# Dunni3/keypoint-diffusion

Measured on AMD Instinct MI355X. Metric: denoising steps/sec, higher is better.
Workload: dtype f32; 1 GPU; egnn_all_atom dynamics (6 EGNN layers, hidden 256, update_kp_feat; fixed receptor encoder), batch of 64 synthetic 300-atom pockets / 25-atom ligands per GPU, T=500, seeded random-init weights, every step taken from the t=T ligand state; batch_per_gpu=64, n_rec=300, n_lig=25, parallelism=dp1

## Files before the change

### keypoint-diffusion_amd/csrc/egnn.hip

```cpp
#include <string.h>

#include <map>
#include <set>
#include <string>
#include <vector>

#include "egnn_kernels.h"
#include "egnn_wide.h"
#include "mfma_core.h"

using namespace kpd;

namespace {

struct LayerW {
    float *wp_e[4], *wx_e[4], *b_e[4], *wr_e[4], *watt[4];
    float *wp_c[4], *wx_c[4], *b_c[4], *wr_c[4], *w3[4];
    void *wh_e[4], *wh_c[4];
    void *chh_p[2][NSLOT];
    void *wh_a[2], *wh_b[2], *wh_2[2];
    float *wp_p[2][NSLOT], *wx_p[2][NSLOT], *b_p[2][NSLOT];
    float *ch_p[2][NSLOT], *wcol_p[2][NSLOT];
    float *wp_a[2], *wx_a[2], *wp_b[2], *wx_b[2], *b0[2], *wp_2[2], *wx_2[2], *b2[2], *ln_w[2], *ln_b[2];
};

const int kSrcNt[4] = {NT_LIG, NT_KP, NT_LIG, NT_KP};
const int kDstNt[4] = {NT_LIG, NT_LIG, NT_KP, NT_KP};
const int kSrcSlot[4] = {0, 0, 6, 4};
const int kDstSlot[4] = {2, 4, 2, 6};
const char *kEtName[4] = {"ll", "kl", "lk", "kk"};
const char *kNtName[2] = {"lig", "kp"};

std::vector<std::string> split(const std::string &s, char c) {
    std::vector<std::string> out;
    size_t p = 0;
    while (true) {
        size_t q = s.find(c, p);
        out.push_back(s.substr(p, q == std::string::npos ? q : q - p));
        if (q == std::string::npos) break;
        p = q + 1;
    }
    return out;
}

int et_index(const std::string &s) {
    for (int i = 0; i < 4; ++i)
        if (s == kEtName[i]) return i;
    return -1;
}
int nt_index(const std::string &s) {
    for (int i = 0; i < 2; ++i)
        if (s == kNtName[i]) return i;
    return -1;
}

}

struct kpd_egnn {
    kpd_egnn_config cfg;
    int n_et;
    int n_upd;
    bool rec_identity;
    Arena warena, ws;
    std::vector<LayerW> L;
    float *le_W0, *le_b0, *le_W1t, *le_b1;
    float *re_W0, *re_b0, *re_W1t, *re_b1;
    float *de_W0, *de_b0, *de_W1, *de_b1;
    std::set<std::string> expected, loaded;
    bool committed = false;
    int debug_layers = -1;
    bool f16_ok = true;
    float *widen_buf = nullptr;
    int *widen_map = nullptr;
    size_t widen_floats = 0, widen_ints = 0;
    int gemm_mode = 0;
    bool f32_only = false;
    int prune_last = 1;
    bool prof_on = false;
    std::vector<hipEvent_t> prof_ev;
    size_t prof_used = 0;

    int cap_B = 0, cap_lig = 0, cap_kp = 0, cap_kk = 0, cap_ll = 0, cap_kl = 0, cap_maxlig = 0, cap_maxkp = 0;
    int tile_cap = 0, tiles_et_cap[4] = {0, 0, 0, 0};
    float *h[2], *x[2], *P[2];
    float *hn_main[4], *hn_cont[4], *xn_main[4], *xn_cont[4];
    int *bidx[2];
    float *z[2];
    int *meta, *ll_deg, *ll_off, *kl_off, *kl_pg;
    kpd_lig_graph lg;
    int kp_table = 1;
    int tab_rows = 0;
    bool last_table = false;
    int *rowmap = nullptr, *kp_ok = nullptr;
    float *tab_in = nullptr;
    int *tab_bidx = nullptr;
    float *hT = nullptr, *PT = nullptr;
    EgnnWide *wide = nullptr;
};

static kpd_status build_weight_arena(kpd_egnn *m) {
    const kpd_egnn_config &c = m->cfg;
    m->warena.poison_at = 2;
    m->L.assign(c.n_layers, LayerW());
    return carve(m->warena, ARENA_TAIL, [&](Carve &A) {
        for (int i = 0; i < c.n_layers; ++i) {
            LayerW &w = m->L[i];
            const std::string pre = "egnn.conv_layers." + std::to_string(i) + ".";
            for (int et = 0; et < m->n_et; ++et) {
                A(w.wp_e[et], WP_FLOATS); A(w.wx_e[et], HS); A(w.b_e[et], HS); A(w.wr_e[et], HS); A(w.watt[et], HS);
                A(w.wp_c[et], WP_FLOATS); A(w.wx_c[et], HS); A(w.b_c[et], HS); A(w.wr_c[et], HS); A(w.w3[et], HS);
                A.as<unsigned short>(w.wh_e[et], WH_HALVES); A.as<unsigned short>(w.wh_c[et], WH_HALVES);
                for (int var = 0; var < 2; ++var) {
                    const int ss = kSrcSlot[et] + var, ds = kDstSlot[et] + var;
                    A(w.wp_p[kSrcNt[et]][ss], WP_FLOATS); A(w.wx_p[kSrcNt[et]][ss], HS);
                    A(w.wp_p[kDstNt[et]][ds], WP_FLOATS); A(w.wx_p[kDstNt[et]][ds], HS); A(w.b_p[kDstNt[et]][ds], HS);
                    A(w.ch_p[kSrcNt[et]][ss], 16 * 4096); A(w.wcol_p[kSrcNt[et]][ss], HS);
                    A(w.ch_p[kDstNt[et]][ds], 16 * 4096); A(w.wcol_p[kDstNt[et]][ds], HS);
                    A.as<unsigned short>(w.chh_p[kSrcNt[et]][ss], CHH_HALVES);
                    A.as<unsigned short>(w.chh_p[kDstNt[et]][ds], CHH_HALVES);
                }
                const std::string e = kEtName[et];
                for (const char *blk : {"edge_mlp.", "coord_mlp."})
                    for (const char *s : {".0.weight", ".0.bias", ".2.weight", ".2.bias"}) m->expected.insert(pre + blk + e + s);
                m->expected.insert(pre + "coord_mlp." + e + ".4.weight");
                m->expected.insert(pre + "soft_attention." + e + ".0.weight");
                m->expected.insert(pre + "soft_attention." + e + ".0.bias");
            }
            for (int nt = 0; nt < m->n_upd; ++nt) {
                A(w.wp_a[nt], WP_FLOATS); A(w.wx_a[nt], HS); A(w.wp_b[nt], WP_FLOATS); A(w.wx_b[nt], HS); A(w.b0[nt], HS);
                A(w.wp_2[nt], WP_FLOATS); A(w.wx_2[nt], HS); A(w.b2[nt], HS); A(w.ln_w[nt], HS); A(w.ln_b[nt], HS);
                A.as<unsigned short>(w.wh_a[nt], WH_HALVES); A.as<unsigned short>(w.wh_b[nt], WH_HALVES);
                A.as<unsigned short>(w.wh_2[nt], WH_HALVES);
                const std::string n = kNtName[nt];
                for (const char *s : {".0.weight", ".0.bias", ".2.weight", ".2.bias"}) m->expected.insert(pre + "node_mlp." + n + s);
                if (c.norm) {
                    m->expected.insert(pre + "layer_norm." + n + ".weight");
                    m->expected.insert(pre + "layer_norm." + n + ".bias");
                }
            }
        }
        A(m->le_W0, 64 * c.atom_nf); A(m->le_b0, 64);
        A(m->le_W1t, 64 * 256); A(m->le_b1, 256);
        for (const char *s : {"lig_encoder.0.weight", "lig_encoder.0.bias", "lig_encoder.2.weight", "lig_encoder.2.bias",
                              "lig_decoder.0.weight", "lig_decoder.0.bias", "lig_decoder.2.weight", "lig_decoder.2.bias"})
            m->expected.insert(s);
        if (!m->rec_identity) {
            A(m->re_W0, 2 * c.rec_nf * c.rec_nf); A(m->re_b0, 2 * c.rec_nf);
            A(m->re_W1t, 2 * c.rec_nf * 256); A(m->re_b1, 256);
            for (const char *s : {"rec_encoder.0.weight", "rec_encoder.0.bias", "rec_encoder.2.weight", "rec_encoder.2.bias"})
                m->expected.insert(s);
        } else {
            m->re_W0 = m->re_b0 = m->re_W1t = m->re_b1 = nullptr;
        }
        A(m->de_W0, 2 * c.atom_nf * 256); A(m->de_b0, 2 * c.atom_nf);
        A(m->de_W1, 2 * c.atom_nf * c.atom_nf); A(m->de_b1, c.atom_nf);
    });
}

extern "C" kpd_status kpd_egnn_create(const kpd_egnn_config *cfg, kpd_egnn **out) {
    KPD_REQUIRE(cfg && out, KPD_ERR_INVALID, "null argument");
    KPD_REQUIRE(cfg->hidden_nf >= 1 && cfg->hidden_nf <= WIDE_MAX_HID, KPD_ERR_INVALID, "hidden_nf=%d: the HIP path covers 1 .. %d",
                cfg->hidden_nf, WIDE_MAX_HID);
    KPD_REQUIRE(cfg->ll_k >= 0 && cfg->ll_k <= KL_KMAX, KPD_ERR_INVALID, "ll_k=%d outside 0..%d (0 = radius graph)", cfg->ll_k, KL_KMAX);
    KPD_REQUIRE(cfg->kl_k >= 0 && cfg->kl_k <= KL_KMAX, KPD_ERR_INVALID, "kl_k=%d outside 0..%d (0 = radius graph)", cfg->kl_k, KL_KMAX);
    KPD_REQUIRE(cfg->kl_k > 0 || cfg->kl_cutoff > 0.0f, KPD_ERR_INVALID, "kl_k = 0 needs graph_cutoffs['kl'] > 0");
    KPD_REQUIRE(cfg->ll_k > 0 || cfg->ll_cutoff > 0.0f, KPD_ERR_INVALID, "ll_k = 0 needs graph_cutoffs['ll'] > 0");
    KPD_REQUIRE(cfg->n_layers >= 1 && cfg->n_layers <= 64, KPD_ERR_INVALID, "n_layers=%d", cfg->n_layers);
    KPD_REQUIRE(cfg->atom_nf >= 1 && cfg->atom_nf <= 256, KPD_ERR_INVALID, "atom_nf=%d outside 1..256", cfg->atom_nf);
    KPD_REQUIRE(cfg->rec_nf >= 1 && cfg->rec_nf <= 256, KPD_ERR_INVALID, "rec_nf=%d outside 1..256", cfg->rec_nf);
    KPD_REQUIRE(cfg->message_norm >= 0.0f, KPD_ERR_INVALID, "message_norm=%f", cfg->message_norm);
    kpd_status st = egnn_kernels_init();
    if (st != KPD_OK) return st;
    kpd_egnn *m = new kpd_egnn();
    m->cfg = *cfg;
    if (cfg->hidden_nf > HID) {
        st = wide_create(*cfg, &m->wide);
        if (st != KPD_OK) {
            delete m;
            return st;
        }
        *out = m;
        return KPD_OK;
    }
    m->n_et = cfg->update_kp_feat ? 4 : 2;
    m->n_upd = cfg->update_kp_feat ? 2 : 1;
    m->rec_identity = cfg->rec_nf == cfg->hidden_nf;
    m->f32_only = cfg->atom_nf > 32 || (m->rec_identity ? cfg->hidden_nf != HID : cfg->rec_nf > 128 && cfg->rec_nf != HID);
    if (const char *e = getenv("KPD_GEMM")) m->gemm_mode = !strcmp(e, "f16x2") && !m->f32_only ? 1 : 0;
    st = build_weight_arena(m);
    if (st == KPD_OK && cfg->hidden_nf != HID) {
        m->widen_floats = (size_t)HW * (2 * HW + 1);
        m->widen_ints = (size_t)HW + 2 * HW + 1;
        if (hipMalloc(reinterpret_cast<void **>(&m->widen_buf), m->widen_floats * 4) != hipSuccess ||
            hipMalloc(reinterpret_cast<void **>(&m->widen_map), m->widen_ints * 4) != hipSuccess) {
            set_error("allocation of the weight staging buffer failed");
            st = KPD_ERR_HIP;
        }
    }
    if (st != KPD_OK) {
        kpd_egnn_destroy(m);
        return st;
    }
    *out = m;
    return KPD_OK;
}

extern "C" void kpd_egnn_destroy(kpd_egnn *m) {
    if (!m) return;
    wide_destroy(m->wide);
    for (hipEvent_t e : m->prof_ev) (void)hipEventDestroy(e);
    if (m->widen_buf) (void)hipFree(m->widen_buf);
    if (m->widen_map) (void)hipFree(m->widen_map);
    m->warena.release();
    m->ws.release();
    delete m;
}

static kpd_status expect_shape(const char *name, const int64_t *shape, int ndim, std::initializer_list<int64_t> want) {
    bool ok = ndim == (int)want.size();
    int i = 0;
    for (int64_t w : want) {
        if (ok && shape[i] != w) ok = false;
        ++i;
    }
    if (!ok) {
        std::string got, exp;
        for (int j = 0; j < ndim; ++j) got += std::to_string(shape[j]) + (j + 1 < ndim ? "," : "");
        for (int64_t w : want) exp += std::to_string(w) + ",";
        set_error("weight %s has shape [%s], expected [%s]", name, got.c_str(), exp.c_str());
        return KPD_ERR_WEIGHTS;
// ... 246 lines not shown
    if (m->wide) return wide_reserve(m->wide, max_B, max_n_lig, max_n_kp, max_n_kk, max_lig_pg, max_kp_pg);
    if (max_B <= m->cap_B && max_n_lig <= m->cap_lig && max_n_kp <= m->cap_kp && max_n_kk <= m->cap_kk &&
        max_lig_pg <= m->cap_maxlig && max_kp_pg <= m->cap_maxkp)
        return KPD_OK;
    max_B = std::max(max_B, m->cap_B); max_n_lig = std::max(max_n_lig, m->cap_lig); max_n_kp = std::max(max_n_kp, m->cap_kp);
    max_n_kk = std::max(max_n_kk, m->cap_kk); max_lig_pg = std::max(max_lig_pg, m->cap_maxlig); max_kp_pg = std::max(max_kp_pg, m->cap_maxkp);
    kpd_lig_graph &g = m->lg;
    KPD_TRY(lig_graph_caps(m->cfg.ll_k, m->cfg.kl_k, max_n_lig, max_n_kp, max_lig_pg, g));
    KPD_REQUIRE(((long)std::max(max_n_lig, max_n_kp) + TM) * NSLOT * HS * 4 < (1l << 32), KPD_ERR_CAPACITY,
                "batch of %d / %d nodes exceeds the 4 GB addressable per node type by the edge kernel's 32-bit row offsets (split the batch)",
                max_n_lig, max_n_kp);
    const int cap_ll = g.cap_ll, cap_kl = g.cap_kl;
    const int E_cap[4] = {cap_ll, cap_kl, cap_kl, std::max(max_n_kk, 1)};
    int tiles[4], tile_cap = 0;
    for (int et = 0; et < 4; ++et) {
        tiles[et] = cdiv(E_cap[et], 32) + 1;
        tile_cap += tiles[et];
    }
    const int n[2] = {max_n_lig, max_n_kp};
    const int rec_nf = m->cfg.rec_nf;
    const int tab_rows = m->rec_identity ? 0 : (int)std::min<long>((long)max_B * rec_nf, max_n_kp / 2);
    KPD_TRY(carve(m->ws, ARENA_TAIL, [&](Carve &W) {
        for (int nt = 0; nt < 2; ++nt) {
            W(m->h[nt], (size_t)(n[nt] + TM) * HS);
            W(m->x[nt], (size_t)n[nt] * 3);
            W.rows(m->P[nt], (size_t)(n[nt] + TM) * NSLOT, HS, HW);
            W(m->bidx[nt], n[nt]);
            W(m->z[nt], max_B);
        }
        for (int et = 0; et < 4; ++et) {
            W.rows(m->hn_main[et], n[kDstNt[et]], HS, HW);
            W.rows(m->hn_cont[et], tiles[et], HS, HW);
            W(m->xn_main[et], (size_t)n[kDstNt[et]] * 4);
            W(m->xn_cont[et], (size_t)tiles[et] * 4);
        }
        carve_lig_graph(W, m->meta, m->ll_deg, m->ll_off, m->kl_off, m->kl_pg, g, max_B, max_n_lig, max_n_kp);
        if (tab_rows > 0) {
            W(m->rowmap, max_n_kp);
            W(m->kp_ok, 1);
            W(m->tab_in, (size_t)tab_rows * rec_nf);
            W(m->tab_bidx, tab_rows);
            W(m->hT, (size_t)(tab_rows + TM) * HS);
            W.rows(m->PT, (size_t)(tab_rows + TM) * NSLOT, HS, HW);
        }
    }));
    m->tab_rows = tab_rows;
    m->last_table = false;
    if (tab_rows > 0) {
        std::vector<float> in((size_t)tab_rows * rec_nf, 0.0f);
        std::vector<int> gi(tab_rows);
        for (int r = 0; r < tab_rows; ++r) {
            in[(size_t)r * rec_nf + r % rec_nf] = 1.0f;
            gi[r] = r / rec_nf;
        }
        KPD_HIP(hipMemcpy(m->tab_in, in.data(), in.size() * 4, hipMemcpyHostToDevice));
        KPD_HIP(hipMemcpy(m->tab_bidx, gi.data(), gi.size() * 4, hipMemcpyHostToDevice));
    }
    for (int et = 0; et < 4; ++et) m->tiles_et_cap[et] = tiles[et];
    m->cap_B = max_B; m->cap_lig = max_n_lig; m->cap_kp = max_n_kp; m->cap_kk = max_n_kk;
    m->cap_ll = cap_ll; m->cap_kl = cap_kl; m->cap_maxlig = max_lig_pg; m->cap_maxkp = max_kp_pg;
    m->tile_cap = tile_cap;
    return KPD_OK;
}

extern "C" kpd_status kpd_egnn_forward(kpd_egnn *m, const kpd_batch *bt, const float *t_dev, float *eps_h, float *eps_x,
                                       void *stream) {
    KPD_REQUIRE(m && bt && t_dev && eps_h && eps_x, KPD_ERR_INVALID, "null argument");
    KPD_REQUIRE(m->wide || m->committed, KPD_ERR_STATE, "kpd_egnn_forward before kpd_egnn_commit");
    KPD_REQUIRE(bt->B >= 1 && bt->n_lig >= 1 && bt->n_kp >= 1, KPD_ERR_INVALID, "empty batch (B=%d n_lig=%d n_kp=%d)", bt->B, bt->n_lig, bt->n_kp);
    KPD_REQUIRE(!m->cfg.update_kp_feat || bt->n_kk == 0 || (bt->kk_src && bt->kk_dst), KPD_ERR_INVALID, "kk edges missing");
    KPD_REQUIRE(bt->kk_rowptr, KPD_ERR_INVALID, "kk_rowptr missing");
    if (m->wide) return wide_forward(m->wide, bt, t_dev, eps_h, eps_x, static_cast<hipStream_t>(stream));
    KPD_REQUIRE(bt->B <= m->cap_B && bt->n_lig <= m->cap_lig && bt->n_kp <= m->cap_kp && bt->n_kk <= m->cap_kk &&
                    bt->max_lig <= m->cap_maxlig && bt->max_kp <= m->cap_maxkp,
                KPD_ERR_CAPACITY, "batch (B=%d lig=%d kp=%d kk=%d maxlig=%d maxkp=%d) exceeds reserved workspace (%d %d %d %d %d %d)",
                bt->B, bt->n_lig, bt->n_kp, bt->n_kk, bt->max_lig, bt->max_kp, m->cap_B, m->cap_lig, m->cap_kp, m->cap_kk,
                m->cap_maxlig, m->cap_maxkp);
    hipStream_t st = static_cast<hipStream_t>(stream);
    const kpd_egnn_config &c = m->cfg;

    const int n_tab = bt->B * c.rec_nf;
    const bool kp_tab = m->kp_table && m->gemm_mode == 0 && m->tab_rows > 0 && (long)bt->B * c.rec_nf <= bt->n_kp / 2;
    m->last_table = kp_tab;
    KPD_TRY(launch_node_graph_index(bt->lig_ptr, bt->B, bt->n_lig, m->bidx[NT_LIG], st, kp_tab ? m->kp_ok : nullptr));
    if (kp_tab)
        KPD_TRY(launch_node_graph_index(bt->kp_ptr, bt->B, bt->n_kp, m->bidx[NT_KP], st, nullptr, bt->kp_h, c.rec_nf, m->rowmap, m->kp_ok));
    else
        KPD_TRY(launch_node_graph_index(bt->kp_ptr, bt->B, bt->n_kp, m->bidx[NT_KP], st));
    const float *x_cur[2] = {bt->lig_x, bt->kp_x};
    KPD_TRY(launch_lig_graph(bt, c.ll_cutoff, c.ll_k, c.kl_cutoff, c.kl_k, &m->lg, m->ll_deg, m->ll_off, m->kl_off, m->kl_pg, st));
    const int tr = TM;
    const int active = c.update_kp_feat ? 0xF : 0x3;
    const bool prune = c.update_kp_feat && m->prune_last;
    const int active_last = prune ? 0x3 : active;
    KPD_TRY(launch_egnn_meta(m->lg.counts, bt->n_kk, active, active_last, bt->lig_ptr, bt->kp_ptr, m->lg.ll_per_graph,
                             bt->kk_rowptr, bt->B, m->kl_off, c.message_norm, c.update_kp_feat, m->meta, m->z[NT_LIG],
                             m->z[NT_KP], st, tr));
    KPD_TRY(launch_embed(bt->lig_h, bt->n_lig, c.atom_nf, m->le_W0, m->le_b0, 64, m->le_W1t, m->le_b1, t_dev,
                         m->bidx[NT_LIG], m->h[NT_LIG], 0, st));
    KPD_TRY(launch_embed(bt->kp_h, bt->n_kp, c.rec_nf, m->re_W0, m->re_b0, 2 * c.rec_nf, m->re_W1t, m->re_b1, t_dev,
                         m->bidx[NT_KP], m->h[NT_KP], m->rec_identity ? 1 : 0, st));
    if (kp_tab) {
        KPD_REQUIRE(n_tab <= m->tab_rows, KPD_ERR_CAPACITY, "internal: %d class rows, table of %d", n_tab, m->tab_rows);
        KPD_TRY(launch_embed(m->tab_in, n_tab, c.rec_nf, m->re_W0, m->re_b0, 2 * c.rec_nf, m->re_W1t, m->re_b1, t_dev, m->tab_bidx,
                             m->hT, 0, st));
    }

    const int e_kl_cap = bt->n_kp * (c.kl_k > 0 ? c.kl_k : std::min(bt->max_lig, 100));
    const int E_cap[4] = {std::max<int>((long)bt->n_lig * std::min(bt->max_lig - 1, c.ll_k > 0 ? c.ll_k : 200), 1), e_kl_cap, e_kl_cap,
                          bt->n_kk};
    int tile_cap = 0, tile_cap_last = 0;
    for (int et = 0; et < m->n_et; ++et) {
        tile_cap += cdiv(E_cap[et], tr);
        if ((active_last >> et) & 1) tile_cap_last += cdiv(E_cap[et], tr);
    }

    const int n[2] = {bt->n_lig, bt->n_kp};
    const int *esrc[4] = {m->lg.ll_src, m->lg.kl_src, m->lg.lk_src, bt->kk_src};
    const int *edst[4] = {m->lg.ll_dst, m->lg.kl_dst, m->lg.lk_dst, bt->kk_dst};
    const int *rowptr[4] = {m->lg.ll_rowptr, m->lg.kl_rowptr, m->lg.lk_rowptr, bt->kk_rowptr};
    const int n_layers = m->debug_layers >= 0 ? std::min(m->debug_layers, c.n_layers) : c.n_layers;

    auto slot_mask = [&](int etmask, int nt) {
        int mk = 0;
        for (int et = 0; et < 4; ++et)
            if ((etmask >> et) & 1) {
                if (kSrcNt[et] == nt) mk |= 3 << kSrcSlot[et];
                if (kDstNt[et] == nt) mk |= 3 << kDstSlot[et];
            }
        return mk;
    };
    auto layer_etmask = [&](int li) { return li == n_layers - 1 ? active_last : active; };
    for (int li = 0; li < n_layers; ++li) {
        const LayerW &L = m->L[li];
        {
            {
                ProjPair pp;
                memset(&pp, 0, sizeof(pp));
                for (int nt = 0; nt < 2; ++nt) {
                    ProjArgs &pa = pp.nt[nt];
                    pa.h = m->h[nt]; pa.n = n[nt]; pa.P = m->P[nt];
                    int k = 0;
                    const int mk = slot_mask(layer_etmask(li), nt);
                    for (int s = 0; s < NSLOT; ++s)
                        if (L.wp_p[nt][s] && ((mk >> s) & 1)) {
                            pa.wp[k] = L.wp_p[nt][s]; pa.wx[k] = L.wx_p[nt][s]; pa.bias[k] = L.b_p[nt][s]; pa.slot[k] = s;
                            pa.chain[k] = L.ch_p[nt][s]; pa.wcol[k] = L.wcol_p[nt][s]; pa.chain_h[k] = L.chh_p[nt][s];
                            ++k;
                        }
                    pp.n_slots[nt] = k;
                }
                pp.tiles0 = cdiv(n[0], TM);
                pp.gemm_mode = m->gemm_mode;
                if (kp_tab && li == 0) {
                    ProjPair pk = pp;
                    pk.n_slots[NT_LIG] = 0;
                    pk.skip_if = m->kp_ok;
                    ProjArgs &pa = pp.nt[NT_KP];
                    pa.h = m->hT; pa.n = n_tab; pa.P = m->PT;
                    KPD_TRY(launch_proj_chain(pp, st));
                    KPD_TRY(launch_proj_chain(pk, st));
                } else {
                    KPD_TRY(launch_proj_chain(pp, st));
                }
            }
        }
        EdgeArgs ea;
        memset(&ea, 0, sizeof(ea));
        const bool last = li == n_layers - 1;
        ea.meta = last ? m->meta + 16 : m->meta;
        ea.x[0] = x_cur[0]; ea.x[1] = x_cur[1]; ea.P[0] = m->P[0]; ea.P[1] = m->P[1];
        ea.use_tanh = c.use_tanh; ea.coords_range = c.coords_range;
        ea.tile_rows = tr;
        ea.gemm_mode = tr == TM ? m->gemm_mode : 0;
        for (int et = 0; et < 4; ++et) {
            ea.src[et] = esrc[et]; ea.dst[et] = edst[et];
            ea.src_nt[et] = kSrcNt[et]; ea.dst_nt[et] = kDstNt[et]; ea.src_slot[et] = kSrcSlot[et]; ea.dst_slot[et] = kDstSlot[et];
            ea.wr_e[et] = L.wr_e[et]; ea.wr_c[et] = L.wr_c[et];
            ea.wp_e[et] = L.wp_e[et]; ea.wx_e[et] = L.wx_e[et]; ea.b_e[et] = L.b_e[et];
            ea.wp_c[et] = L.wp_c[et]; ea.wx_c[et] = L.wx_c[et]; ea.b_c[et] = L.b_c[et];
            ea.wh_e[et] = L.wh_e[et]; ea.wh_c[et] = L.wh_c[et];
            ea.watt[et] = L.watt[et]; ea.w3[et] = L.w3[et];
            ea.hn_main[et] = m->hn_main[et]; ea.hn_cont[et] = m->hn_cont[et];
            ea.xn_main[et] = m->xn_main[et]; ea.xn_cont[et] = m->xn_cont[et];
        }
        if (kp_tab && li == 0) { ea.PT = m->PT; ea.rowmap = m->rowmap; ea.kp_ok = m->kp_ok; }
        const bool prof = m->prof_on && m->prof_used + 2 <= m->prof_ev.size();
        if (prof) KPD_HIP(hipEventRecord(m->prof_ev[m->prof_used], st));
        KPD_TRY(launch_egnn_edge(ea, last ? tile_cap_last : tile_cap, st));
        if (prof) {
            KPD_HIP(hipEventRecord(m->prof_ev[m->prof_used + 1], st));
            m->prof_used += 2;
        }
        auto fill_update = [&](NodeArgs &na, int nt) {
            na.n = n[nt]; na.h = m->h[nt]; na.x = m->x[nt]; na.bidx = m->bidx[nt]; na.z = m->z[nt];
            int k = 0;
            for (int et = 0; et < m->n_et; ++et)
                if (kDstNt[et] == nt && ((layer_etmask(li) >> et) & 1)) {
                    na.rowptr[k] = rowptr[et];
                    na.hn_main[k] = m->hn_main[et]; na.hn_cont[k] = m->hn_cont[et];
                    na.xn_main[k] = m->xn_main[et]; na.xn_cont[k] = m->xn_cont[et];
                    ++k;
                }
            na.n_in = k;
            na.wp_a = L.wp_a[nt]; na.wx_a = L.wx_a[nt]; na.wp_b = L.wp_b[nt]; na.wx_b = L.wx_b[nt]; na.b0 = L.b0[nt];
            na.wp_2 = L.wp_2[nt]; na.wx_2 = L.wx_2[nt]; na.b2 = L.b2[nt]; na.ln_w = L.ln_w[nt]; na.ln_b = L.ln_b[nt];
            na.ln_inv_n = 1.0f / (float)(c.hidden_nf + 1); na.ln_pad = (float)(HID - c.hidden_nf);
            na.wh_a = L.wh_a[nt]; na.wh_b = L.wh_b[nt]; na.wh_2 = L.wh_2[nt];
            na.norm = c.norm;
            na.tile_shift = 6;
        };
        {
            NodeLayerPair lp;
            memset(&lp, 0, sizeof(lp));
            for (int nt = 0; nt < 2; ++nt) {
                NodeLayerArgs &na = lp.nt[nt];
                na.u.n = n[nt]; na.u.h = m->h[nt];
                if (nt < m->n_upd && !(nt == NT_KP && last && prune)) {
                    fill_update(na.u, nt);
                    na.u.x_in = x_cur[nt] == m->x[nt] ? nullptr : x_cur[nt];
                    na.do_update = 1;
                }
                if (!na.do_update && !na.do_proj) na.u.n = 0;
            }
            lp.tiles0 = cdiv(lp.nt[0].u.n, TN);
            lp.gemm_mode = m->gemm_mode;
            KPD_TRY(launch_node_layer(lp, st));
            for (int nt = 0; nt < 2; ++nt)
                if (lp.nt[nt].do_update) x_cur[nt] = m->x[nt];
        }
    }
    if (x_cur[NT_LIG] != m->x[NT_LIG]) KPD_HIP(hipMemcpyAsync(m->x[NT_LIG], bt->lig_x, (size_t)bt->n_lig * 12, hipMemcpyDeviceToDevice, st));
    if (x_cur[NT_KP] != m->x[NT_KP]) KPD_HIP(hipMemcpyAsync(m->x[NT_KP], bt->kp_x, (size_t)bt->n_kp * 12, hipMemcpyDeviceToDevice, st));
    KPD_TRY(launch_decode(m->h[NT_LIG], m->x[NT_LIG], bt->lig_x, bt->n_lig, c.atom_nf, 2 * c.atom_nf, m->de_W0, m->de_b0,
                          m->de_W1, m->de_b1, eps_h, eps_x, st));
    return KPD_OK;
}

extern "C" kpd_status kpd_egnn_debug_state(kpd_egnn *m, const char *what, float *out, int64_t n_floats, void *stream) {
    KPD_REQUIRE(m && what && out, KPD_ERR_INVALID, "null argument");
    hipStream_t st = static_cast<hipStream_t>(stream);
    if (m->wide) return wide_debug_state(m->wide, what, out, n_floats, st);
    const std::string w(what);
    const float *src = nullptr;
    if (w == "h_lig") src = m->h[0];
    else if (w == "h_kp") src = m->h[1];
    else if (w == "x_lig") src = m->x[0];
    else if (w == "x_kp") src = m->x[1];
    else if (w == "z_lig") src = m->z[0];
    else if (w == "z_kp") src = m->z[1];
    else if (w.size() == 4 && (w.rfind("xnm", 0) == 0 || w.rfind("xnc", 0) == 0 || w.rfind("hnm", 0) == 0 || w.rfind("hnc", 0) == 0) &&
             w[3] >= '0' && w[3] < '4') {
        const int et = w[3] - '0';
        src = w[0] == 'x' ? (w[2] == 'm' ? m->xn_main[et] : m->xn_cont[et]) : (w[2] == 'm' ? m->hn_main[et] : m->hn_cont[et]);
    }
    else if (w == "kp_table_ok") {
        KPD_REQUIRE(n_floats == 1, KPD_ERR_INVALID, "kp_table_ok is one value");
        if (!m->last_table) {
            KPD_HIP(hipMemsetAsync(out, 0, 4, st));
            return KPD_OK;
        }
        src = reinterpret_cast<const float *>(m->kp_ok);
    } else if (w.rfind("kp_table=", 0) == 0) {
        m->kp_table = atoi(w.c_str() + 9);
        return KPD_OK;
    }
    else if (w.rfind("layers=", 0) == 0) {
        m->debug_layers = atoi(w.c_str() + 7);
        return KPD_OK;
    } else if (w.rfind("prune=", 0) == 0) {
        m->prune_last = atoi(w.c_str() + 6);
        return KPD_OK;
    } else if (w.rfind("gemm=", 0) == 0) {
        const std::string v = w.substr(5);
        KPD_REQUIRE(v == "f32" || v == "f16x2", KPD_ERR_INVALID, "gemm mode must be f32 or f16x2");
        KPD_REQUIRE(v == "f32" || !m->f32_only, KPD_ERR_INVALID,
                    "gemm=f16x2: atom_nf = %d / rec_nf = %d (hidden_nf = %d) run the exact fp32 path only; the f16x2 mode covers atom_nf <= 32 "
                    "with rec_nf <= 128 or 256, or the identity keypoint encoder at hidden_nf 256", m->cfg.atom_nf, m->cfg.rec_nf, m->cfg.hidden_nf);
        KPD_REQUIRE(v == "f32" || !m->committed || m->f16_ok, KPD_ERR_WEIGHTS, "%s", F16_RANGE_ERROR);
        m->gemm_mode = v == "f16x2" ? 1 : 0;
        return KPD_OK;
    }
    KPD_REQUIRE(src, KPD_ERR_INVALID, "unknown debug tap '%s'", what);
    KPD_HIP(hipMemcpyAsync(out, src, (size_t)n_floats * 4, hipMemcpyDeviceToDevice, st));
    return KPD_OK;
}

extern "C" kpd_status kpd_egnn_profile(kpd_egnn *m, int32_t enable) {
    KPD_REQUIRE(m, KPD_ERR_INVALID, "null handle");
    KPD_REQUIRE(!m->wide, KPD_ERR_INVALID, "kpd_egnn_profile times the fused edge kernel of hidden_nf <= 256; hidden_nf = %d has none",
                m->cfg.hidden_nf);
    if (enable && m->prof_ev.empty()) {
        m->prof_ev.resize(2 * 8192);
        for (hipEvent_t &e : m->prof_ev) KPD_HIP(hipEventCreate(&e));
    }
    m->prof_on = enable != 0;
    m->prof_used = 0;
    return KPD_OK;
}

extern "C" kpd_status kpd_egnn_profile_read(kpd_egnn *m, double *total_ms, int32_t *launches) {
    KPD_REQUIRE(m && total_ms && launches, KPD_ERR_INVALID, "null argument");
    KPD_REQUIRE(!m->wide, KPD_ERR_INVALID, "kpd_egnn_profile_read: no fused edge kernel at hidden_nf = %d", m->cfg.hidden_nf);
    double tot = 0.0;
    for (size_t i = 0; i + 1 < m->prof_used; i += 2) {
        KPD_HIP(hipEventSynchronize(m->prof_ev[i + 1]));
        float ms = 0.0f;
        KPD_HIP(hipEventElapsedTime(&ms, m->prof_ev[i], m->prof_ev[i + 1]));
        tot += ms;
    }
    *total_ms = tot;
    *launches = (int32_t)(m->prof_used / 2);
    return KPD_OK;
}

extern "C" kpd_status kpd_egnn_last_counts(kpd_egnn *m, int32_t out[8], void *stream) {
    KPD_REQUIRE(m && out, KPD_ERR_INVALID, "null argument");
    if (m->wide) return wide_last_counts(m->wide, out, static_cast<hipStream_t>(stream));
    for (int i = 0; i < 7; ++i) out[i] = 0;
    out[7] = m->gemm_mode;
    if (!m->ws.base) return KPD_OK;
    hipStream_t st = static_cast<hipStream_t>(stream);
    int host[25];
    KPD_HIP(hipMemcpyAsync(host, m->meta, sizeof(host), hipMemcpyDeviceToHost, st));
    KPD_HIP(hipStreamSynchronize(st));
    for (int i = 0; i < 4; ++i) out[i] = host[i];
    out[4] = host[8];
    out[5] = host[16 + 8];
    out[6] = host[16] + host[17] + host[18] + host[19];
    return KPD_OK;
}

extern "C" kpd_status kpd_build_lig_graph(const kpd_batch *bt, float ll_cutoff, int32_t ll_k, float kl_cutoff, int32_t kl_k,
                                          const kpd_lig_graph *out, void *stream) {
    KPD_REQUIRE(bt && out, KPD_ERR_INVALID, "null argument");
    hipStream_t st = static_cast<hipStream_t>(stream);
    int *tmp = nullptr;
    const size_t cnt = (size_t)bt->n_lig + 3 * ((size_t)bt->B + 2);
    KPD_HIP(hipMalloc(reinterpret_cast<void **>(&tmp), cnt * sizeof(int)));
    kpd_status s = launch_lig_graph(bt, ll_cutoff, ll_k, kl_cutoff, kl_k, out, tmp, tmp + bt->n_lig, tmp + bt->n_lig + bt->B + 2,
                                    tmp + bt->n_lig + 2 * (bt->B + 2), st);
    hipError_t e = hipStreamSynchronize(st);
    (void)hipFree(tmp);
    if (s != KPD_OK) return s;
    KPD_HIP(e);
    return KPD_OK;
}
```

### keypoint-diffusion_amd/csrc/egnn_chain.hip

```cpp
#include <algorithm>
#include <cstdlib>

#include "chain_core.h"
#include "egnn_kernels.h"

namespace kpd {

namespace {

constexpr int ENT = 16;
constexpr int ECH4 = ENT * 64;

__device__ __forceinline__ float reduce_q(float v) {
    v += __shfl_xor(v, 16);
    v += __shfl_xor(v, 32);
    return v;
}

}

struct ProjWs {
    ProjPair p;
    int blocks0;
    int bpc[2];
    int tpb;
};

constexpr int WS_TILE = 128;
constexpr int WS_W4 = 16 * 8 * 64;
constexpr int WS_LDS_BYTES = WS_W4 * 16 + (128 + 128 + HS) * 4;

__global__ __launch_bounds__(512, 1) void k_proj_ws(ProjWs qa) {
    extern __shared__ __attribute__((aligned(16))) float smem[];
    v4f *W = reinterpret_cast<v4f *>(smem);
    float *s_wcol = smem + WS_W4 * 4, *s_bias = s_wcol + 128, *s_wrow = s_bias + 128;
    const int tid = threadIdx.x, wave = tid >> 6, lane = tid & 63;
    if (qa.p.skip_if && *qa.p.skip_if) return;
    const int which = (int)blockIdx.x >= qa.blocks0 ? 1 : 0;
    const ProjArgs &a = qa.p.nt[which];
    const int local = blockIdx.x - (which ? qa.blocks0 : 0);
    const int combo = local / qa.bpc[which], chunk = local - combo * qa.bpc[which];
    const int s = combo >> 1, hf = combo & 1;
    const int tiles = (a.n + WS_TILE - 1) / WS_TILE;
    const int t0 = chunk * qa.tpb, t1 = min(tiles, t0 + qa.tpb);
    if (t0 >= t1) return;
    {
        const v4f *src = reinterpret_cast<const v4f *>(a.chain[s]);
#pragma unroll
        for (int j = 0; j < WS_W4 / 512; ++j) {
            const int i = tid + 512 * j, ks = i >> 9, rem = i & 511;
            W[i] = src[(size_t)ks * ECH4 + 8 * hf * 64 + rem];
        }
        const float *bias = a.bias[s];
        if (tid < 128) {
            s_wcol[tid] = a.wcol[s][128 * hf + tid];
            s_bias[tid] = bias ? bias[128 * hf + tid] : 0.0f;
        }
        for (int i = tid; i < HS; i += 512) s_wrow[i] = i <= 256 ? a.wx[s][i] : 0.0f;
    }
    __syncthreads();
    const int el = lane & 15, q = lane >> 4;
    const float bias256 = a.bias[s] ? a.bias[s][256] : 0.0f;
    auto load_x = [&](int t, v4f (&x)[ENT], float &x256) {
        const int row = min(t * WS_TILE + 16 * wave + el, a.n - 1);
        const float *hrow = a.h + (size_t)row * HS;
#pragma unroll
        for (int nt = 0; nt < ENT; ++nt) x[nt] = *reinterpret_cast<const v4f *>(hrow + 16 * nt + 4 * q);
        x256 = hrow[256];
    };
    auto store_tile = [&](const v4f (&acc)[8], int row, float out256) {
        if (row >= 0 && row < a.n) {
            float *orow = a.P + ((size_t)row * NSLOT + a.slot[s]) * HS + 128 * hf;
#pragma unroll
            for (int m = 0; m < 8; ++m) *reinterpret_cast<v4f *>(orow + 16 * m + 4 * q) = acc[m];
            if (hf == 0 && q == 0) orow[256] = out256;
        }
    };
    v4f x[ENT], xn[ENT], accp[8];
    float h256, h256n, out256p = 0.0f;
    int rowp = -1;
#pragma unroll
    for (int m = 0; m < 8; ++m) accp[m] = zero4();
    load_x(t0, xn, h256n);
#pragma unroll 1
    for (int t = t0; t < t1; ++t) {
#pragma unroll
        for (int nt = 0; nt < ENT; ++nt)
#pragma unroll
            for (int r = 0; r < 4; ++r) asm volatile("v_mov_b32 %0, %1" : "=v"(x[nt][r]) : "v"(xn[nt][r]));
        asm volatile("v_mov_b32 %0, %1" : "=v"(h256) : "v"(h256n));
        __builtin_amdgcn_sched_barrier(0);
        store_tile(accp, rowp, out256p);
        if (t + 1 < t1) load_x(t + 1, xn, h256n);
        v4f acc[8];
#pragma unroll
        for (int m = 0; m < 8; ++m)
            acc[m] = h256 * *reinterpret_cast<const v4f *>(s_wcol + 16 * m + 4 * q) + *reinterpret_cast<const v4f *>(s_bias + 16 * m + 4 * q);
        float part = 0.0f;
        if (hf == 0) {
#pragma unroll
            for (int nt = 0; nt < ENT; ++nt) {
                const v4f wv = *reinterpret_cast<const v4f *>(s_wrow + 16 * nt + 4 * q);
                part += x[nt][0] * wv[0] + x[nt][1] * wv[1] + x[nt][2] * wv[2] + x[nt][3] * wv[3];
            }
        }
        const v4f *wp = W + lane;
        v4f w[2][4];
#pragma unroll
        for (int m = 0; m < 4; ++m) w[0][m] = wp[m * 64];
#pragma unroll
        for (int b = 0; b < 32; ++b) {
            if (b + 1 < 32) {
#pragma unroll
                for (int m = 0; m < 4; ++m) w[(b + 1) & 1][m] = wp[(4 * (b + 1) + m) * 64];
            }
            __builtin_amdgcn_sched_barrier(0);
            const v4f xin = x[b >> 1];
            const int g = b & 1;
#pragma unroll
            for (int r = 0; r < 4; ++r)
#pragma unroll
                for (int m = 0; m < 4; ++m) acc[4 * g + m] = mfma16(w[b & 1][m][r], xin[r], acc[4 * g + m]);
            __builtin_amdgcn_sched_barrier(0);
        }
        const int row = t * WS_TILE + 16 * wave + el;
        const float out256 = hf == 0 ? reduce_q(part) + bias256 + h256 * s_wrow[256] : 0.0f;
#pragma unroll
        for (int m = 0; m < 8; ++m) accp[m] = acc[m];
        rowp = row;
        out256p = out256;
    }
    store_tile(accp, rowp, out256p);
}

__global__ __launch_bounds__(512, 1) void k_proj_ws_h(ProjWs qa) {
    extern __shared__ __attribute__((aligned(16))) float smem[];
    f32x4 *W = reinterpret_cast<f32x4 *>(smem);
    float *s_wcol = smem + WS_W4 * 4, *s_bias = s_wcol + 128, *s_wrow = s_bias + 128;
    const int tid = threadIdx.x, wave = tid >> 6, lane = tid & 63;
    const int which = (int)blockIdx.x >= qa.blocks0 ? 1 : 0;
    const ProjArgs &a = qa.p.nt[which];
    const int local = blockIdx.x - (which ? qa.blocks0 : 0);
    const int combo = local / qa.bpc[which], chunk = local - combo * qa.bpc[which];
    const int s = combo >> 1, hf = combo & 1;
    const int tiles = (a.n + WS_TILE - 1) / WS_TILE;
    const int t0 = chunk * qa.tpb, t1 = min(tiles, t0 + qa.tpb);
    if (t0 >= t1) return;
    {
        const f32x4 *src = reinterpret_cast<const f32x4 *>(a.chain_h[s]);
#pragma unroll
        for (int j = 0; j < WS_W4 / 512; ++j) {
            const int i = tid + 512 * j, kb = i >> 10, rem = i & 1023;
            W[i] = src[(size_t)(kb * 16 + 8 * hf) * 128 + rem];
        }
        const float *bias = a.bias[s];
        if (tid < 128) {
            s_wcol[tid] = a.wcol[s][128 * hf + tid];
            s_bias[tid] = bias ? bias[128 * hf + tid] : 0.0f;
        }
        for (int i = tid; i < HS; i += 512) s_wrow[i] = i <= 256 ? a.wx[s][i] : 0.0f;
    }
    __syncthreads();
    const int el = lane & 15, q = lane >> 4;
    const float bias256 = a.bias[s] ? a.bias[s][256] : 0.0f;
    auto load_x = [&](int t, v4f (&x)[16], float &x256) {
        const int row = min(t * WS_TILE + 16 * wave + el, a.n - 1);
        const float *hrow = a.h + (size_t)row * HS + 8 * q;
#pragma unroll
        for (int kb = 0; kb < 8; ++kb) {
            x[2 * kb] = *reinterpret_cast<const v4f *>(hrow + 32 * kb);
            x[2 * kb + 1] = *reinterpret_cast<const v4f *>(hrow + 32 * kb + 4);
        }
        x256 = hrow[256 - 8 * q];
    };
    auto store_tile = [&](const v4f (&acc)[8], int row) {
        if (row >= 0 && row < a.n) {
            float *orow = a.P + ((size_t)row * NSLOT + a.slot[s]) * HS + 128 * hf;
#pragma unroll
            for (int m = 0; m < 8; ++m) *reinterpret_cast<v4f *>(orow + 16 * m + 4 * q) = acc[m];
        }
    };
    v4f xn[16], accp[8];
    f32x4 xh[8], xl[8];
    float h256n;
    int rowp = -1;
#pragma unroll
    for (int m = 0; m < 8; ++m) accp[m] = zero4();
    load_x(t0, xn, h256n);
#pragma unroll 1
    for (int t = t0; t < t1; ++t) {
        const float h256 = h256n;
        float part = 0.0f;
#pragma unroll
        for (int kb = 0; kb < 8; ++kb) {
            const v4f u = xn[2 * kb], v = xn[2 * kb + 1];
            if (hf == 0) {
                const v4f w0 = *reinterpret_cast<const v4f *>(s_wrow + 32 * kb + 8 * q), w1 = *reinterpret_cast<const v4f *>(s_wrow + 32 * kb + 8 * q + 4);
                part += u[0] * w0[0] + u[1] * w0[1] + u[2] * w0[2] + u[3] * w0[3] + v[0] * w1[0] + v[1] * w1[1] + v[2] * w1[2] + v[3] * w1[3];
            }
            unsigned h0, h1, h2, h3, l0, l1, l2, l3;
            split_pair(H_SCALE_A * u[0], H_SCALE_A * u[1], h0, l0);
            split_pair(H_SCALE_A * u[2], H_SCALE_A * u[3], h1, l1);
            split_pair(H_SCALE_A * v[0], H_SCALE_A * v[1], h2, l2);
            split_pair(H_SCALE_A * v[2], H_SCALE_A * v[3], h3, l3);
            typedef unsigned u32x4 __attribute__((ext_vector_type(4)));
            xh[kb] = __builtin_bit_cast(f32x4, u32x4{h0, h1, h2, h3});
            xl[kb] = __builtin_bit_cast(f32x4, u32x4{l0, l1, l2, l3});
        }
        __builtin_amdgcn_sched_barrier(0);
        store_tile(accp, rowp);
        if (t + 1 < t1) load_x(t + 1, xn, h256n);
        const int row = t * WS_TILE + 16 * wave + el;
        if (hf == 0) {
            const float out256 = reduce_q(part) + bias256 + h256 * s_wrow[256];
            if (q == 0 && row < a.n) a.P[((size_t)row * NSLOT + a.slot[s]) * HS + 256] = out256;
        }
        v4f acc[8];
#pragma unroll
        for (int m = 0; m < 8; ++m)
            acc[m] = (1.0f / H_UNSCALE) * (h256 * *reinterpret_cast<const v4f *>(s_wcol + 16 * m + 4 * q) + *reinterpret_cast<const v4f *>(s_bias + 16 * m + 4 * q));
        const f32x4 *wp = W + lane;
        f32x4 w[3][4];
#pragma unroll
        for (int i = 0; i < 4; ++i) w[0][i] = wp[i * 64];
#pragma unroll
        for (int b = 0; b < 32; ++b) {
            if (b + 1 < 32) {
#pragma unroll
                for (int i = 0; i < 4; ++i) w[(b + 1) % 3][i] = wp[(4 * (b + 1) + i) * 64];
            }
            __builtin_amdgcn_sched_barrier(0);
            const int kb = b >> 2, m0 = 2 * (b & 3);
            const f32x4 *wb = w[b % 3];
            acc[m0] = __builtin_amdgcn_mfma_f32_16x16x32_f16(as_h8(wb[1]), as_h8(xh[kb]), acc[m0], 0, 0, 0);
            acc[m0 + 1] = __builtin_amdgcn_mfma_f32_16x16x32_f16(as_h8(wb[3]), as_h8(xh[kb]), acc[m0 + 1], 0, 0, 0);
            acc[m0] = __builtin_amdgcn_mfma_f32_16x16x32_f16(as_h8(wb[0]), as_h8(xl[kb]), acc[m0], 0, 0, 0);
            acc[m0 + 1] = __builtin_amdgcn_mfma_f32_16x16x32_f16(as_h8(wb[2]), as_h8(xl[kb]), acc[m0 + 1], 0, 0, 0);
            acc[m0] = __builtin_amdgcn_mfma_f32_16x16x32_f16(as_h8(wb[0]), as_h8(xh[kb]), acc[m0], 0, 0, 0);
            acc[m0 + 1] = __builtin_amdgcn_mfma_f32_16x16x32_f16(as_h8(wb[2]), as_h8(xh[kb]), acc[m0 + 1], 0, 0, 0);
            __builtin_amdgcn_sched_barrier(0);
        }
#pragma unroll
        for (int m = 0; m < 8; ++m) accp[m] = H_UNSCALE * acc[m];
        rowp = row;
    }
    store_tile(accp, rowp);
}

kpd_status launch_proj_chain(const ProjPair &p, hipStream_t st) {
    const int slots = std::max(p.n_slots[0], p.n_slots[1]);
    if (poison_level() >= 1) KPD_TRY(poison_lds(st));
    if (slots == 0) return KPD_OK;
    for (int nt = 0; nt < 2; ++nt)
        for (int s = 0; s < p.n_slots[nt]; ++s)
            KPD_REQUIRE(p.nt[nt].chain[s] && p.nt[nt].wcol[s], KPD_ERR_STATE, "projection slot %d not packed", s);
    KPD_TRY(ensure_dynamic_lds(reinterpret_cast<const void *>(k_proj_ws), WS_LDS_BYTES));
    const int target = cu_count();
    ProjWs q;
    q.p = p;
    int units = 0, tl[2];
    for (int nt = 0; nt < 2; ++nt) {
        tl[nt] = p.n_slots[nt] ? cdiv(p.nt[nt].n, WS_TILE) : 0;
        units += 2 * p.n_slots[nt] * tl[nt];
    }
    if (units == 0) return KPD_OK;
    int blocks[2];
    for (q.tpb = std::max(1, cdiv(units, target));; ++q.tpb) {
        for (int nt = 0; nt < 2; ++nt) {
            q.bpc[nt] = std::max(1, cdiv(tl[nt], q.tpb));
            blocks[nt] = tl[nt] ? 2 * p.n_slots[nt] * q.bpc[nt] : 0;
        }
        if (blocks[0] + blocks[1] <= target || q.tpb >= std::max(tl[0], tl[1])) break;
    }
    q.blocks0 = blocks[0];
    if (p.gemm_mode == 1) {
        KPD_REQUIRE(!p.skip_if, KPD_ERR_INVALID, "projection launch: skip_if is served by the exact mode only");
        for (int nt = 0; nt < 2; ++nt)
            for (int s = 0; s < p.n_slots[nt]; ++s)
                KPD_REQUIRE(p.nt[nt].chain_h[s], KPD_ERR_STATE, "projection slot %d has no f16 planes (f16x2 mode)", s);
        KPD_TRY(ensure_dynamic_lds(reinterpret_cast<const void *>(k_proj_ws_h), WS_LDS_BYTES));
        hipLaunchKernelGGL(k_proj_ws_h, dim3(blocks[0] + blocks[1]), dim3(512), WS_LDS_BYTES, st, q);
        KPD_LAUNCH_CHECK();
        return KPD_OK;
    }
    hipLaunchKernelGGL(k_proj_ws, dim3(blocks[0] + blocks[1]), dim3(512), WS_LDS_BYTES, st, q);
    KPD_LAUNCH_CHECK();
    return KPD_OK;
}

}
```

### keypoint-diffusion_amd/csrc/egnn_kernels.h

```cpp
#pragma once
#include "engine.h"

namespace kpd {

constexpr int NSLOT = 8;
constexpr int ATT_BIAS_AT = 260;
constexpr int BIAS_K = 260;
constexpr int ET_LL = 0, ET_KL = 1, ET_LK = 2, ET_KK = 3;
constexpr int NT_LIG = 0, NT_KP = 1;

constexpr int EDGE_LDS_BYTES = TM * SA * 4 + (TM * 2 + TM + 3 * TM + TM + 3 * TM + 4 * HS + 8 + TM) * 4;
constexpr int EDGE_H_LDS_BYTES = 64 * 280 * 2 * 2 + (TM * 2 + TM + 3 * TM + TM + 3 * TM + 2 * HS + 8) * 4 + 2 * 2 * 272 * 2;

struct ProjArgs {
    const float *h;
    int n;
    float *P;
    const float *wp[NSLOT];
    const float *wx[NSLOT];
    const float *bias[NSLOT];
    int slot[NSLOT];
    const float *chain[NSLOT];
    const float *wcol[NSLOT];
    const void *chain_h[NSLOT];
};

struct ProjPair {
    ProjArgs nt[2];
    int tiles0;
    int n_slots[2];
    int slots_per_block;
    int gemm_mode;
    const int *skip_if;
};

struct EdgeArgs {
    const int *meta;
    const int *src[4];
    const int *dst[4];
    const float *x[2];
    const float *P[2];
    int src_nt[4], dst_nt[4], src_slot[4], dst_slot[4];
    const float *wr_e[4], *wr_c[4];
    const float *wp_e[4], *wx_e[4], *b_e[4];
    const float *wp_c[4], *wx_c[4], *b_c[4];
    const float *watt[4];
    const float *w3[4];
    float *hn_main[4], *hn_cont[4];
    float *xn_main[4], *xn_cont[4];
    int use_tanh;
    float coords_range;
    const void *wh_e[4], *wh_c[4];
    int gemm_mode;
    int tile_rows;
    int split_slots;
    const float *PT;
    const int *rowmap;
    const int *kp_ok;
};

struct EdgeTrainArgs {
    const int *meta;
    const int *src[4];
    const int *dst[4];
    const float *x[2];
    const float *P[2];
    int src_nt[4], dst_nt[4];
    int slot[4][2][2];
    const float *wr[4][2], *wp[4][2], *wx[4][2];
    const float *watt[4], *w3[4];
    float *hn_main[4], *hn_cont[4], *xn_main[4], *xn_cont[4];
    int use_tanh;
    float coords_range;
    float *keep[4][2][4];
    float *att[4], *sc[4], *dij[4], *xdiff[4], *nvec[4];
};

struct EdgePackEntry {
    const float *W1, *W2, *b2;
    const float *head, *head_b;
    float *wp, *wx, *wr, *head_out;
};
struct EdgePackTab {
    EdgePackEntry e[8];
    int n;
    int transposed;
};

struct EdgeBwdArgs {
    const int *meta;
    const int *dst[4];
    int dst_nt[4];
    const float *dhn[2];
    const float *dxo[2];
    const float *zinv[2];
    float *keep[4][2][4];
    float *att[4], *sc[4], *nvec[4];
    const float *dij[4];
    const float *wa[4], *w3[4];
    const float *wpT[4][2], *wxT[4][2], *wr[4][2];
    float *dv_main[4][2], *dv_cont[4][2], *dvw_main[4][2], *dvw_cont[4][2];
    float *part[2];
    int part_ld;
    int use_tanh;
    float coords_range;
};

struct NodeArgs {
    int n;
    float *h;
    float *x;
    const float *x_in;
    const int *bidx;
    const float *z;
    int n_in;
    const int *rowptr[2];
    const float *hn_main[2], *hn_cont[2];
    const float *xn_main[2], *xn_cont[2];
    const float *wp_a, *wx_a, *wp_b, *wx_b, *b0;
    const float *wp_2, *wx_2, *b2;
    const void *wh_a, *wh_b, *wh_2;
    const float *ln_w, *ln_b;
    int norm;
    float ln_inv_n, ln_pad;
    int tile_shift;
};

struct NodeLayerArgs {
    NodeArgs u;
    int do_update, do_proj;
    float *P;
    int n_slots;
    const float *wp[NSLOT], *wx[NSLOT], *bias[NSLOT];
    int slot[NSLOT];
};

struct NodeLayerPair {
    NodeLayerArgs nt[2];
    int tiles0;
    int gemm_mode;
};

constexpr int TN = 32;
constexpr int NODE_LAYER_LDS_BYTES = TN * SA * 4 + 3 * TN * 4 + 3 * HS * 4;
constexpr int NODE_H_TILE_FLOATS = 2 * TN * 280 / 2;
constexpr int NODE_H_LDS_BYTES = NODE_H_TILE_FLOATS * 4 + 3 * TN * 4;


kpd_status egnn_kernels_init();
kpd_status launch_node_graph_index(const int *ptr, int B, int n, int *bidx, hipStream_t st, int *set_ok = nullptr,
                                   const float *kp_h = nullptr, int fin = 0, int *rowmap = nullptr, int *ok = nullptr);
kpd_status launch_egnn_meta(const int *counts, int e_kk, int active_mask, int active_last, const int *lig_ptr, const int *kp_ptr,
                            const int *ll_per_graph, const int *kk_rowptr, int B, const int *kl_off, float message_norm,
                            int update_kp, int *meta, float *z_lig, float *z_kp, hipStream_t st, int tile_rows = TM);
kpd_status launch_embed(const float *in, int n, int fin, const float *W0, const float *b0, int hid, const float *W1t,
                        const float *b1, const float *t, const int *bidx, float *out, int identity, hipStream_t st);
kpd_status launch_decode(const float *h, const float *x, const float *x0, int n, int atom_nf, int hid, const float *W0,
                         const float *b0, const float *W1, const float *b1, float *eps_h, float *eps_x, hipStream_t st);
kpd_status launch_egnn_edge(const EdgeArgs &a, int tile_cap, hipStream_t st);
kpd_status launch_egnn_edge_train(const EdgeTrainArgs &a, int tile_cap, hipStream_t st);
struct EdgePiecesSumArgs {
    const float *hn_main[4], *hn_cont[4], *xn_main[4], *xn_cont[4];
    const int *rowptr[4];
    int live[4], dst_nt[4];
    const float *zinv[2];
    int n[2];
    float *hn[2], *xn[2];
};
kpd_status launch_edge_pieces_sum(const EdgePiecesSumArgs &a, hipStream_t st);
kpd_status launch_edge_train_pack(const EdgePackTab &t, hipStream_t st);
kpd_status launch_egnn_edge_bwd(const EdgeBwdArgs &a, int tile_cap, hipStream_t st);
struct EdgePiecesBatch {
    struct One {
        const float *m1, *c1, *m2, *c2;
        const int *rowptr;
        int n;
        float *o1, *o2;
    } e[8];
    int ldo;
};
kpd_status launch_edge_pieces_set(const EdgePiecesBatch &b, int count, hipStream_t st);
kpd_status launch_proj_chain(const ProjPair &p, hipStream_t st);
kpd_status launch_node_layer(const NodeLayerPair &p, hipStream_t st);

}
```

Measured before the change: 157.4 steps/s.

## Balance projection work evenly across workgroups using fine-grained unit ranges

The fp32 projection kernel now splits its work into 64-row units, with weight-refill cost counted as extra units, and gives each workgroup an equal contiguous range of them. A range may cross several slot/half combos, so a workgroup reloads the weight chunk into LDS between segments. Waves stride over 16-row groups instead of fixed 128-row tiles. The goal is to remove load imbalance and tail effects from the old per-combo chunking, at the cost of extra weight reloads and syncs in blocks that span combos. New debug knobs and P taps are added, and even mode is on by default.

```diff
diff --git a/keypoint-diffusion_amd/csrc/egnn.hip b/keypoint-diffusion_amd/csrc/egnn.hip
--- a/keypoint-diffusion_amd/csrc/egnn.hip
+++ b/keypoint-diffusion_amd/csrc/egnn.hip
@@ -76,6 +76,8 @@
     int gemm_mode = 0;
     bool f32_only = false;
     int prune_last = 1;
+    int proj_even = 1, proj_wgs = 0;
+    int proj_refill = 1;
     bool prof_on = false;
     std::vector<hipEvent_t> prof_ev;
     size_t prof_used = 0;
@@ -628,6 +630,7 @@
                 }
                 pp.tiles0 = cdiv(n[0], TM);
                 pp.gemm_mode = m->gemm_mode;
+                pp.proj_even = m->proj_even; pp.proj_wgs = m->proj_wgs; pp.proj_refill = m->proj_refill;
                 if (kp_tab && li == 0) {
                     ProjPair pk = pp;
                     pk.n_slots[NT_LIG] = 0;
@@ -725,6 +728,8 @@
     else if (w == "x_kp") src = m->x[1];
     else if (w == "z_lig") src = m->z[0];
     else if (w == "z_kp") src = m->z[1];
+    else if (w == "P_lig") src = m->P[0];
+    else if (w == "P_kp") src = m->P[1];
     else if (w.size() == 4 && (w.rfind("xnm", 0) == 0 || w.rfind("xnc", 0) == 0 || w.rfind("hnm", 0) == 0 || w.rfind("hnc", 0) == 0) &&
              w[3] >= '0' && w[3] < '4') {
         const int et = w[3] - '0';
@@ -746,6 +751,15 @@
         return KPD_OK;
     } else if (w.rfind("prune=", 0) == 0) {
         m->prune_last = atoi(w.c_str() + 6);
+        return KPD_OK;
+    } else if (w.rfind("proj_even=", 0) == 0) {
+        m->proj_even = atoi(w.c_str() + 10) != 0;
+        return KPD_OK;
+    } else if (w.rfind("proj_wgs=", 0) == 0) {
+        m->proj_wgs = std::max(0, atoi(w.c_str() + 9));
+        return KPD_OK;
+    } else if (w.rfind("proj_refill=", 0) == 0) {
+        m->proj_refill = std::max(0, atoi(w.c_str() + 12));
         return KPD_OK;
     } else if (w.rfind("gemm=", 0) == 0) {
         const std::string v = w.substr(5);
diff --git a/keypoint-diffusion_amd/csrc/egnn_chain.hip b/keypoint-diffusion_amd/csrc/egnn_chain.hip
--- a/keypoint-diffusion_amd/csrc/egnn_chain.hip
+++ b/keypoint-diffusion_amd/csrc/egnn_chain.hip
@@ -24,31 +24,28 @@
     int blocks0;
     int bpc[2];
     int tpb;
+    int even;
+    int refill;
+    int groups[2];
+    int cunits[2];
+    int units0, units;
 };
 
 constexpr int WS_TILE = 128;
 constexpr int WS_W4 = 16 * 8 * 64;
 constexpr int WS_LDS_BYTES = WS_W4 * 16 + (128 + 128 + HS) * 4;
 
-__global__ __launch_bounds__(512, 1) void k_proj_ws(ProjWs qa) {
-    extern __shared__ __attribute__((aligned(16))) float smem[];
+__device__ __forceinline__ void proj_ws_segment(const ProjArgs &a, int s, int hf, int g0, int g1, int wave, float *smem) {
     v4f *W = reinterpret_cast<v4f *>(smem);
     float *s_wcol = smem + WS_W4 * 4, *s_bias = s_wcol + 128, *s_wrow = s_bias + 128;
-    const int tid = threadIdx.x, wave = tid >> 6, lane = tid & 63;
-    if (qa.p.skip_if && *qa.p.skip_if) return;
-    const int which = (int)blockIdx.x >= qa.blocks0 ? 1 : 0;
-    const ProjArgs &a = qa.p.nt[which];
-    const int local = blockIdx.x - (which ? qa.blocks0 : 0);
-    const int combo = local / qa.bpc[which], chunk = local - combo * qa.bpc[which];
-    const int s = combo >> 1, hf = combo & 1;
-    const int tiles = (a.n + WS_TILE - 1) / WS_TILE;
-    const int t0 = chunk * qa.tpb, t1 = min(tiles, t0 + qa.tpb);
-    if (t0 >= t1) return;
+    int lane;
+    asm volatile("v_mbcnt_lo_u32_b32 %0, -1, 0\n\tv_mbcnt_hi_u32_b32 %0, -1, %0" : "=&v"(lane));
+    const int tid = 64 * wave + lane;
     {
         const v4f *src = reinterpret_cast<const v4f *>(a.chain[s]);
 #pragma unroll
         for (int j = 0; j < WS_W4 / 512; ++j) {
-            const int i = tid + 512 * j, ks = i >> 9, rem = i & 511;
+            const int i = tid + 512 * j, ks = j, rem = tid;
             W[i] = src[(size_t)ks * ECH4 + 8 * hf * 64 + rem];
         }
         const float *bias = a.bias[s];
@@ -56,13 +53,13 @@
             s_wcol[tid] = a.wcol[s][128 * hf + tid];
             s_bias[tid] = bias ? bias[128 * hf + tid] : 0.0f;
         }
-        for (int i = tid; i < HS; i += 512) s_wrow[i] = i <= 256 ? a.wx[s][i] : 0.0f;
+        if (tid < HS) s_wrow[tid] = tid <= 256 ? a.wx[s][tid] : 0.0f;
     }
     __syncthreads();
     const int el = lane & 15, q = lane >> 4;
     const float bias256 = a.bias[s] ? a.bias[s][256] : 0.0f;
-    auto load_x = [&](int t, v4f (&x)[ENT], float &x256) {
-        const int row = min(t * WS_TILE + 16 * wave + el, a.n - 1);
+    auto load_x = [&](int g, v4f (&x)[ENT], float &x256) {
+        const int row = min(16 * g + el, a.n - 1);
         const float *hrow = a.h + (size_t)row * HS;
 #pragma unroll
         for (int nt = 0; nt < ENT; ++nt) x[nt] = *reinterpret_cast<const v4f *>(hrow + 16 * nt + 4 * q);
@@ -81,9 +78,11 @@
     int rowp = -1;
 #pragma unroll
     for (int m = 0; m < 8; ++m) accp[m] = zero4();
-    load_x(t0, xn, h256n);
+    const int gw = g0 + wave;
+    if (gw >= g1) return;
+    load_x(gw, xn, h256n);
 #pragma unroll 1
-    for (int t = t0; t < t1; ++t) {
+    for (int g = gw; g < g1; g += 8) {
 #pragma unroll
         for (int nt = 0; nt < ENT; ++nt)
 #pragma unroll
@@ -91,7 +90,7 @@
         asm volatile("v_mov_b32 %0, %1" : "=v"(h256) : "v"(h256n));
         __builtin_amdgcn_sched_barrier(0);
         store_tile(accp, rowp, out256p);
-        if (t + 1 < t1) load_x(t + 1, xn, h256n);
+        if (g + 8 < g1) load_x(g + 8, xn, h256n);
         v4f acc[8];
 #pragma unroll
         for (int m = 0; m < 8; ++m)
@@ -123,7 +122,7 @@
                 for (int m = 0; m < 4; ++m) acc[4 * g + m] = mfma16(w[b & 1][m][r], xin[r], acc[4 * g + m]);
             __builtin_amdgcn_sched_barrier(0);
         }
-        const int row = t * WS_TILE + 16 * wave + el;
+        const int row = 16 * g + el;
         const float out256 = hf == 0 ? reduce_q(part) + bias256 + h256 * s_wrow[256] : 0.0f;
 #pragma unroll
         for (int m = 0; m < 8; ++m) accp[m] = acc[m];
@@ -131,6 +130,38 @@
         out256p = out256;
     }
     store_tile(accp, rowp, out256p);
+}
+
+__global__ __launch_bounds__(512, 1) void k_proj_ws(ProjWs qa) {
+    extern __shared__ __attribute__((aligned(16))) float smem[];
+    if (qa.p.skip_if && *qa.p.skip_if) return;
+    const int wave = __builtin_amdgcn_readfirstlane(threadIdx.x >> 6);
+    int u0, u1;
+    if (qa.even) {
+        const unsigned w = blockIdx.x, nw = gridDim.x, base = (unsigned)qa.units / nw, rem = (unsigned)qa.units - base * nw;
+        u0 = (int)(w * base + w * rem / nw);
+        u1 = (int)((w + 1) * base + (w + 1) * rem / nw);
+    } else {
+        const int which = (int)blockIdx.x >= qa.blocks0 ? 1 : 0;
+        const int local = blockIdx.x - (which ? qa.blocks0 : 0);
+        const int combo = local / qa.bpc[which], chunk = local - combo * qa.bpc[which];
+        const int C = qa.cunits[which], base = (which ? qa.units0 : 0) + combo * C;
+        u0 = base + min(C, chunk * qa.tpb * (WS_TILE / 64));
+        u1 = base + min(C, (chunk + 1) * qa.tpb * (WS_TILE / 64));
+    }
+    bool filled = false;
+#pragma unroll 1
+    for (int u = u0; u < u1;) {
+        const int which = u >= qa.units0 ? 1 : 0;
+        const int C = qa.cunits[which], ul = u - (which ? qa.units0 : 0);
+        const int combo = ul / C, c0 = ul - combo * C, c1 = min(C, c0 + (u1 - u));
+        u += c1 - c0;
+        const int g0 = 4 * max(0, c0 - qa.refill), g1 = min(qa.groups[which], 4 * (c1 - qa.refill));
+        if (g0 >= g1) continue;
+        if (filled) __syncthreads();
+        proj_ws_segment(qa.p.nt[which], combo >> 1, combo & 1, g0, g1, wave, smem);
+        filled = true;
+    }
 }
 
 __global__ __launch_bounds__(512, 1) void k_proj_ws_h(ProjWs qa) {
@@ -264,6 +295,21 @@
         units += 2 * p.n_slots[nt] * tl[nt];
     }
     if (units == 0) return KPD_OK;
+    q.even = p.gemm_mode == 0 && p.proj_even;
+    q.refill = q.even ? std::min(std::max(p.proj_refill, 0), 64) : 0;
+    for (int nt = 0; nt < 2; ++nt) {
+        q.groups[nt] = tl[nt] ? cdiv(p.nt[nt].n, 16) : 0;
+        q.cunits[nt] = tl[nt] ? q.refill + cdiv(q.groups[nt], 4) : 0;
+    }
+    q.units0 = 2 * p.n_slots[0] * q.cunits[0];
+    q.units = q.units0 + 2 * p.n_slots[1] * q.cunits[1];
+    if (q.even) {
+        q.blocks0 = 0; q.bpc[0] = q.bpc[1] = 1; q.tpb = 0;
+        const int wgs = std::min(std::min(p.proj_wgs > 0 ? p.proj_wgs : target, q.units), 32767);
+        hipLaunchKernelGGL(k_proj_ws, dim3(wgs), dim3(512), WS_LDS_BYTES, st, q);
+        KPD_LAUNCH_CHECK();
+        return KPD_OK;
+    }
     int blocks[2];
     for (q.tpb = std::max(1, cdiv(units, target));; ++q.tpb) {
         for (int nt = 0; nt < 2; ++nt) {
diff --git a/keypoint-diffusion_amd/csrc/egnn_kernels.h b/keypoint-diffusion_amd/csrc/egnn_kernels.h
--- a/keypoint-diffusion_amd/csrc/egnn_kernels.h
+++ b/keypoint-diffusion_amd/csrc/egnn_kernels.h
@@ -32,6 +32,9 @@
     int slots_per_block;
     int gemm_mode;
     const int *skip_if;
+    int proj_even;
+    int proj_wgs;
+    int proj_refill;
 };
 
 struct EdgeArgs {
```

Result: no change. 158.3 steps/s, median of 6 (+0.6%).
